# RiccZamboni/mepol

Measured on AMD Instinct MI355X. Metric: MEPOL epoch wall-clock (C3: N=200000, d=29, k=30; rollout excluded), lower is better.
Workload: dtype f64; 1 GPU; C3 Ant-shaped MEPOL epoch (k-NN + off-policy loop + final H); particles=200000, num_traj=400, traj_len=500, d=29, k=30, policy=29->[400, 300]->8 f64, parallelism=dp1

## Files before the change

### mepol_amd/csrc/policy_fwd.hip

```cpp
#include "mfma_f64.hpp"

namespace mepol {
namespace pfwd {

using mfma::d4;
using mfma::head_epilogue;
using mfma::kLog2Pi;
using mfma::kStdEps;

constexpr int BM = 64, BN = 320;
constexpr int WC = 4;
constexpr int FR = 2, FC = 5;
constexpr int kThreads = 512;
constexpr int KT = 16, KP = 18;
constexpr int CB = BN * (KT / 2), PB = CB / kThreads;
constexpr int kAChunk = 8;
static_assert(CB % kThreads == 0, "W2 k-tile chunks must divide the block");
static_assert(kThreads == BM * kAChunk, "head_epilogue: one thread per (row, action slot)");

template <int FP>
constexpr size_t lds_bytes() {
  return (2ull * BM * KP + 2ull * BN * KP + (size_t)(BM + 2 * KT) * (FP + 2)) * sizeof(double);
}

template <int FP, bool VEC>
__global__ __launch_bounds__(kThreads) void policy_fwd_kernel(
    const double* __restrict__ x, int64_t N, int F, const double* __restrict__ W1,
    const double* __restrict__ b1, int H1, const double* __restrict__ W2,
    const double* __restrict__ b2, int H2, const double* __restrict__ Wm,
    const double* __restrict__ bm, const double* __restrict__ log_std,
    const double* __restrict__ act, int A, double* __restrict__ h1_out,
    double* __restrict__ z2_out, double* __restrict__ mu_out, double* __restrict__ logp_out,
    uint16_t* __restrict__ mask_out) {
  constexpr int XP = FP + 2;
  extern __shared__ double lds[];
  double* sA = lds;
  double* sB = sA + 2 * BM * KP;
  double* sX = sB + 2 * BN * KP;
  double* sW = sX + BM * XP;
  const int tid = threadIdx.x, lane = tid & 63, wave = tid >> 6;
  const int wr = wave / WC, wc = wave % WC;
  const int fr = lane & 15, g = lane >> 4;
  const int64_t row0 = (int64_t)blockIdx.x * BM;
  const int nkt = (H1 + KT - 1) / KT;

  for (int e = tid; e < BM * FP; e += kThreads) {
    const int r = e / FP, f = e % FP;
    const int64_t rr = min<int64_t>(row0 + r, N - 1);
    const double v = x[rr * F + min(f, F - 1)];
    sX[r * XP + f] = (f < F && row0 + r < N) ? v : 0.0;
  }

  constexpr int PW = (KT * FP + kThreads - 1) / kThreads;
  double rw[PW];
  auto w1_load = [&](int kt) __attribute__((always_inline)) {
#pragma unroll
    for (int p = 0; p < PW; ++p) {
      const int e = tid + p * kThreads, r = e / FP, f = e % FP;
      rw[p] = W1[(int64_t)min(kt * KT + r, H1 - 1) * F + min(f, F - 1)];
    }
  };
  auto w1_store = [&](int kt) __attribute__((always_inline)) {
#pragma unroll
    for (int p = 0; p < PW; ++p) {
      const int e = tid + p * kThreads, r = e / FP, f = e % FP;
      if (e < KT * FP) sW[((kt & 1) * KT + r) * XP + f] = (kt * KT + r < H1 && f < F) ? rw[p] : 0.0;
    }
  };
  auto h1_gen = [&](int kt, int buf) __attribute__((always_inline)) {
    constexpr int NS = FP / 4, NCH = NS < 4 ? NS : 4;
    d4 hc[NCH];
#pragma unroll
    for (int u = 0; u < NCH; ++u) hc[u] = d4{0.0, 0.0, 0.0, 0.0};
    const double* xr = sX + (wave * 16 + fr) * XP + g;
    const double* wr1 = sW + ((kt & 1) * KT + fr) * XP + g;
#pragma unroll
    for (int s = 0; s < NS; ++s)
      hc[s % NCH] = __builtin_amdgcn_mfma_f64_16x16x4f64(xr[4 * s], wr1[4 * s], hc[s % NCH], 0,
                                                         0, 0);
    d4 h = hc[0];
#pragma unroll
    for (int u = 1; u < NCH; ++u) h += hc[u];
    const int c = kt * KT + fr;
    const double bc = c < H1 ? b1[c] : 0.0;
    const int mw = (H1 + 15) / 16;
#pragma unroll
    for (int q = 0; q < 4; ++q) {
      const int r = wave * 16 + g + 4 * q;
      const double v = c < H1 ? fmax(h[q] + bc, 0.0) : 0.0;
      sA[(buf * BM + r) * KP + fr] = v;
      if (c < H1 && row0 + r < N) h1_out[(row0 + r) * H1 + c] = v;
      const uint64_t bits = __ballot(v > 0.0);
      if (mask_out && fr == 0 && row0 + r < N)
        mask_out[(row0 + r) * mw + kt] = (uint16_t)(bits >> (16 * g));
    }
  };

  double2 rb[PB];
  auto b_load = [&](int kt) __attribute__((always_inline)) {
#pragma unroll
    for (int p = 0; p < PB; ++p) {
      const int ch = tid + p * kThreads, r = ch >> 3, k = kt * KT + 2 * (ch & 7);
      const double* row = W2 + (int64_t)min(r, H2 - 1) * H1;
      double2 v;
      if constexpr (VEC)
        v = *reinterpret_cast<const double2*>(row + min(k, H1 - 2));
      else
        v = double2{row[min(k, H1 - 1)], row[min(k + 1, H1 - 1)]};
      rb[p] = v;
    }
  };
  auto b_store = [&](int kt, int buf) __attribute__((always_inline)) {
#pragma unroll
    for (int p = 0; p < PB; ++p) {
      const int ch = tid + p * kThreads, r = ch >> 3, k = kt * KT + 2 * (ch & 7);
      double2 v = rb[p];
      if (r >= H2 || k >= H1) v = double2{0.0, 0.0};
      if (k + 1 >= H1) v.y = 0.0;
      *reinterpret_cast<double2*>(sB + (buf * BN + r) * KP + 2 * (ch & 7)) = v;
    }
  };

  d4 acc[FR][FC];
#pragma unroll
  for (int i = 0; i < FR; ++i)
#pragma unroll
    for (int j = 0; j < FC; ++j) acc[i][j] = d4{0.0, 0.0, 0.0, 0.0};

  b_load(0);
  w1_load(0);
  w1_store(0);
  if (nkt > 1) {
    w1_load(1);
    w1_store(1);
  }
  __syncthreads();
  if (wave < 4) h1_gen(0, 0);
  b_store(0, 0);
  __syncthreads();
  for (int kt = 0; kt < nkt; ++kt) {
    const int buf = kt & 1;
    if (kt + 1 < nkt) {
      b_load(kt + 1);
      if (kt + 2 < nkt) w1_load(kt + 2);
      if (wave < 4) h1_gen(kt + 1, buf ^ 1);
    }
    double2 a[FR][2], b[FC][2];
#pragma unroll
    for (int i = 0; i < FR; ++i) {
      const double* p = sA + (buf * BM + wr * FR * 16 + i * 16 + fr) * KP + 4 * g;
      a[i][0] = *reinterpret_cast<const double2*>(p);
      a[i][1] = *reinterpret_cast<const double2*>(p + 2);
    }
#pragma unroll
    for (int j = 0; j < FC; ++j) {
      const double* p = sB + (buf * BN + wc * FC * 16 + j * 16 + fr) * KP + 4 * g;
      b[j][0] = *reinterpret_cast<const double2*>(p);
      b[j][1] = *reinterpret_cast<const double2*>(p + 2);
    }
#pragma unroll
    for (int s = 0; s < 4; ++s) {
#pragma unroll
      for (int i = 0; i < FR; ++i) {
        const double av = (s & 1) ? a[i][s >> 1].y : a[i][s >> 1].x;
#pragma unroll
        for (int j = 0; j < FC; ++j) {
          const double bv = (s & 1) ? b[j][s >> 1].y : b[j][s >> 1].x;
          acc[i][j] = __builtin_amdgcn_mfma_f64_16x16x4f64(av, bv, acc[i][j], 0, 0, 0);
        }
      }
    }
    if (kt + 1 < nkt) {
      b_store(kt + 1, buf ^ 1);
      if (kt + 2 < nkt) w1_store(kt + 2);
    }
    __syncthreads();
  }

  head_epilogue<FR, FC, kAChunk, WC, BM>(acc, row0, wr * FR * 16, wc, N, b2, H2, Wm, bm, log_std,
                                         act, A, z2_out, mu_out, logp_out, sB);
}

template <int FP, int RG>
__global__ __launch_bounds__(256) void layer1_kernel(const double* __restrict__ x, int64_t N,
                                                     int F, const double* __restrict__ W1,
                                                     const double* __restrict__ b1, int H1,
                                                     double* __restrict__ h1_out,
                                                     uint16_t* __restrict__ mask_out) {
  constexpr int NS = FP / 4;
  const int l = threadIdx.x & 63, fr = l & 15, g = l >> 4;
  const int64_t r0 = ((int64_t)blockIdx.x * 4 + (threadIdx.x >> 6)) * 16 * RG;
  if (r0 >= N) return;
  double xv[RG][NS];
#pragma unroll
  for (int rg = 0; rg < RG; ++rg) {
    const int64_t xr = min<int64_t>(r0 + 16 * rg + fr, N - 1);
#pragma unroll
    for (int s = 0; s < NS; ++s) {
      const int f = 4 * s + g;
      const double v = x[xr * F + min(f, F - 1)];
      xv[rg][s] = f < F ? v : 0.0;
    }
  }
  const int nkt = (H1 + 15) / 16, mw = nkt;
  double wv[2][NS], bc[2];
  auto loadw = [&](int b, int kt) __attribute__((always_inline)) {
    const int c = min(kt * 16 + fr, H1 - 1);
    const double* wr = W1 + (int64_t)c * F;
#pragma unroll
    for (int s = 0; s < NS; ++s) {
      const int f = 4 * s + g;
      const double v = wr[min(f, F - 1)];
      wv[b][s] = f < F ? v : 0.0;
    }
    bc[b] = b1[c];
  };
  auto tile = [&](int b, int kt) __attribute__((always_inline)) {
    if (kt + 1 < nkt) loadw(b ^ 1, kt + 1);
    d4 h[RG];
#pragma unroll
    for (int rg = 0; rg < RG; ++rg) h[rg] = d4{0.0, 0.0, 0.0, 0.0};
#pragma unroll
    for (int s = 0; s < NS; ++s)
#pragma unroll
      for (int rg = 0; rg < RG; ++rg)
        h[rg] = __builtin_amdgcn_mfma_f64_16x16x4f64(xv[rg][s], wv[b][s], h[rg], 0, 0, 0);
    const int c = kt * 16 + fr;
#pragma unroll
    for (int rg = 0; rg < RG; ++rg)
#pragma unroll
      for (int q = 0; q < 4; ++q) {
        const int64_t r = r0 + 16 * rg + g + 4 * q;
        const double v = c < H1 ? fmax(h[rg][q] + bc[b], 0.0) : 0.0;
        if (c < H1 && r < N) __builtin_nontemporal_store(v, h1_out + r * H1 + c);
        const uint64_t bits = __ballot(v > 0.0);
        if (mask_out && fr == 0 && r < N) mask_out[r * mw + kt] = (uint16_t)(bits >> (16 * g));
      }
  };
  loadw(0, 0);
  int kt = 0;
#pragma nounroll
  for (; kt + 1 < nkt; kt += 2) {
    tile(0, kt);
    tile(1, kt + 1);
  }
  if (kt < nkt) tile(0, kt);
}

namespace zh {
constexpr int FI = 5, NW = 4, NS = 2;
constexpr int kCUs = 256;
constexpr int kOcc = 2;
inline int pick_tile(int64_t n) {
  for (int tile = 16; tile < 64; tile *= 2)
    if ((n + tile - 1) / tile <= kCUs) return tile;
  return 64;
}
}

template <int FO>
__global__ __launch_bounds__(64 * zh::NW) __attribute__((amdgpu_waves_per_eu(zh::kOcc))) void z2_head_kernel(
    const double* __restrict__ h1, int64_t N, int H1, const double* __restrict__ W2,
    const double* __restrict__ b2, int H2, const double* __restrict__ Wm,
    const double* __restrict__ bm, const double* __restrict__ log_std,
    const double* __restrict__ act, int A, double* __restrict__ z2_out,
    double* __restrict__ mu_out, double* __restrict__ logp_out) {
  constexpr int FI = zh::FI, NW = zh::NW, NS = zh::NS, NL = FO + FI;
  constexpr int ZM = 16 * FO;
  __shared__ double sMu[NW * ZM * 4];
  const int tid = threadIdx.x, l = tid & 63, fr = l & 15, g = l >> 4;
  const int w = __builtin_amdgcn_readfirstlane(tid >> 6);
  const int64_t row0 = (int64_t)blockIdx.x * ZM;
  const int col0 = 16 * FI * w;
  const double* ap[FO];
  const double* bp[FI];
#pragma unroll
  for (int t = 0; t < FO; ++t) ap[t] = h1 + min<int64_t>(row0 + 16 * t + fr, N - 1) * H1 + 2 * g;
#pragma unroll
  for (int u = 0; u < FI; ++u) bp[u] = W2 + (int64_t)min(col0 + 16 * u + fr, H2 - 1) * H1 + 2 * g;
  d4 acc[FO][FI];
#pragma unroll
  for (int t = 0; t < FO; ++t)
#pragma unroll
    for (int u = 0; u < FI; ++u) acc[t][u] = d4{0.0, 0.0, 0.0, 0.0};
  const int nst = (H1 + 7) / 8, nfull = H1 / 8;
  double2 R[NS][NL];
  auto load = [&](double2 (&D)[NL], int st) __attribute__((always_inline)) {
    const int k = min(8 * st, H1 - 2 - 2 * g);
#pragma unroll
    for (int t = 0; t < FO; ++t) D[t] = *reinterpret_cast<const double2*>(ap[t] + k);
#pragma unroll
    for (int u = 0; u < FI; ++u) D[FO + u] = *reinterpret_cast<const double2*>(bp[u] + k);
  };
  auto mma = [&](const double2 (&D)[NL]) __attribute__((always_inline)) {
#pragma unroll
    for (int t = 0; t < FO; ++t)
#pragma unroll
      for (int u = 0; u < FI; ++u)
        acc[t][u] = __builtin_amdgcn_mfma_f64_16x16x4f64(D[t].x, D[FO + u].x, acc[t][u], 0, 0, 0);
#pragma unroll
    for (int t = 0; t < FO; ++t)
#pragma unroll
      for (int u = 0; u < FI; ++u)
        acc[t][u] = __builtin_amdgcn_mfma_f64_16x16x4f64(D[t].y, D[FO + u].y, acc[t][u], 0, 0, 0);
  };
  mfma::ring_k_loop<NS, false>(
      nfull, nst, [&](int p, int st) __attribute__((always_inline)) { load(R[p], st); },
      [&](int p, int st) __attribute__((always_inline)) {
        if (8 * st + 2 * g >= H1) {
#pragma unroll
          for (int v = 0; v < NL; ++v) R[p][v] = double2{0.0, 0.0};
        }
      },
      [&](int p) __attribute__((always_inline)) { mma(R[p]); });

  double b2v[FI];
#pragma unroll
  for (int u = 0; u < FI; ++u) {
    const int c = col0 + 16 * u + fr;
    b2v[u] = c < H2 ? b2[c] : -HUGE_VAL;
#pragma unroll
    for (int t = 0; t < FO; ++t)
#pragma unroll
      for (int q = 0; q < 4; ++q) {
        const int64_t r = row0 + 16 * t + g + 4 * q;
        if (c < H2 && r < N) z2_out[r * H2 + c] = acc[t][u][q];
      }
  }
  constexpr int AC = 4;
  const int er = tid >> 2, ea = tid & 3;
  double lp = 0.0;
  for (int a0 = 0; a0 < A; a0 += AC) {
    double wmv[FI][AC];
#pragma unroll
    for (int u = 0; u < FI; ++u) {
      const int c = col0 + 16 * u + fr;
#pragma unroll
      for (int a = 0; a < AC; ++a)
        wmv[u][a] = (c < H2 && a0 + a < A) ? Wm[(int64_t)(a0 + a) * H2 + c] : 0.0;
    }
#pragma unroll
    for (int t = 0; t < FO; ++t)
#pragma unroll
      for (int q = 0; q < 4; ++q) {
        double p[AC];
#pragma unroll
        for (int a = 0; a < AC; ++a) p[a] = 0.0;
#pragma unroll
        for (int u = 0; u < FI; ++u) {
          const double rv = fmax(acc[t][u][q] + b2v[u], 0.0);
#pragma unroll
          for (int a = 0; a < AC; ++a) p[a] = fma(rv, wmv[u][a], p[a]);
        }
        int comp;
        const double v = mfma::reduce_scatter_g<AC, 16>(p, fr, comp);
        if ((fr & 3) == 0) sMu[(w * ZM + 16 * t + g + 4 * q) * AC + comp] = v;
      }
    __syncthreads();
    {
      const int a = a0 + ea;
      const int64_t r = row0 + er;
      double term = 0.0;
      if (er < ZM && a < A && r < N) {
        double m = sMu[(0 * ZM + er) * AC + ea];
#pragma unroll
        for (int v = 1; v < NW; ++v) m += sMu[(v * ZM + er) * AC + ea];
        m += bm[a];
        const double lsa = log_std[a];
        const double sd = exp(lsa) + kStdEps;
        const double d = act[r * A + a] - m;
        mu_out[r * A + a] = m;
        term = -0.5 * (kLog2Pi + 2.0 * lsa + d * d / (sd * sd));
      }
      term += __shfl_xor(term, 2, kWave);
      term += __shfl_xor(term, 1, kWave);
      lp += term;
    }
    __syncthreads();
  }
  if (ea == 0 && er < ZM && row0 + er < N) logp_out[row0 + er] = lp;
}

#ifndef MEPOL_L1_RG
#define MEPOL_L1_RG 2
#endif
constexpr int kLayer1RowGroups = MEPOL_L1_RG;

template <int FP>
int launch_split(const double* x, int64_t n, int F, const double* W1, const double* b1, int H1,
                 const double* W2, const double* b2, int H2, const double* Wm, const double* bm,
                 const double* log_std, const double* act, int A, double* h1, double* z2,
                 double* mu, double* logp, uint16_t* mask, int row_tile, hipStream_t st) {
  const int tile = row_tile ? row_tile : zh::pick_tile(n);
  const unsigned blocks = (unsigned)((n + tile - 1) / tile);
  constexpr int RG = kLayer1RowGroups;
  hipLaunchKernelGGL((layer1_kernel<FP, RG>), dim3((unsigned)((n + 64 * RG - 1) / (64 * RG))),
                     dim3(256), 0, st, x, n, F, W1, b1, H1, h1, mask);
  MEPOL_CHECK_LAUNCH();
#define MEPOL_Z2(FOV)                                                                       \
  hipLaunchKernelGGL(z2_head_kernel<FOV>, dim3(blocks), dim3(64 * zh::NW), 0, st, h1, n, H1, W2, \
                     b2, H2, Wm, bm, log_std, act, A, z2, mu, logp)
  if (tile == 64)
    MEPOL_Z2(4);
  else if (tile == 32)
    MEPOL_Z2(2);
  else
    MEPOL_Z2(1);
#undef MEPOL_Z2
  MEPOL_CHECK_LAUNCH();
  return 0;
}

template <int FP, bool VEC>
int launch(const double* x, int64_t n, int F, const double* W1, const double* b1, int H1,
           const double* W2, const double* b2, int H2, const double* Wm, const double* bm,
           const double* log_std, const double* act, int A, double* h1, double* z2, double* mu,
           double* logp, uint16_t* mask, hipStream_t st) {
  MEPOL_HIP((max_dynamic_lds<policy_fwd_kernel<FP, VEC>>((int)lds_bytes<FP>())));
  const unsigned blocks = (unsigned)((n + BM - 1) / BM);
  hipLaunchKernelGGL((policy_fwd_kernel<FP, VEC>), dim3(blocks), dim3(kThreads), lds_bytes<FP>(), st,
                     x, n, F, W1, b1, H1, W2, b2, H2, Wm, bm, log_std, act, A, h1, z2, mu, logp,
                     mask);
  MEPOL_CHECK_LAUNCH();
  return 0;
}

}
}

static int policy_forward(const char* who, const double* x, int64_t n, int in_features,
                          const double* W1, const double* b1, int hidden0, const double* W2,
                          const double* b2, int hidden1, const double* Wm, const double* bm,
                          const double* log_std, const double* actions, int action_dim,
                          double* h1_out, double* z2_out, double* mu_out, double* logp_out,
                          uint16_t* h1_mask_out, int row_tile, void* stream) {
  using namespace mepol::pfwd;
  if (n < 0 || in_features <= 0 || in_features > 64 || hidden0 <= 0 || hidden1 <= 0 ||
      hidden1 > BN || action_dim <= 0 || !x || !W1 || !b1 || !W2 || !b2 || !Wm || !bm ||
      !log_std || !actions || !h1_out || !z2_out || !mu_out || !logp_out ||
      ((uintptr_t)W2 & 15)) {
    mepol::set_error("%s: bad arguments (in_features <= 64, hidden1 <= %d)", who, BN);
    return mepol::kErrBadArg;
  }
  if (row_tile != 0 && row_tile != 64 && row_tile != 32 && row_tile != 16) {
    mepol::set_error("%s: row_tile %d (0 = automatic, 64, 32 or 16)", who, row_tile);
    return mepol::kErrBadArg;
  }
  const bool split = hidden0 % 2 == 0 && ((uintptr_t)h1_out & 15) == 0;
  if (!split && row_tile != 0 && row_tile != 64) {
    mepol::set_error("%s: the one-kernel form (odd hidden0) has 64-row blocks only, not %d", who,
                     row_tile);
    return mepol::kErrUnsupported;
  }
  if (n == 0) return 0;
  hipStream_t st = (hipStream_t)stream;
#define MEPOL_PF(FPV)                                                                        \
  {                                                                                          \
  if (split)                                                                                 \
    return launch_split<FPV>(x, n, in_features, W1, b1, hidden0, W2, b2, hidden1, Wm, bm,     \
                             log_std, actions, action_dim, h1_out, z2_out, mu_out, logp_out, \
                             h1_mask_out, row_tile, st);                                     \
  return (hidden0 % 2 == 0 && hidden0 >= 2)                                                  \
             ? launch<FPV, true>(x, n, in_features, W1, b1, hidden0, W2, b2, hidden1, Wm, bm, \
                                 log_std, actions, action_dim, h1_out, z2_out, mu_out,        \
                                 logp_out, h1_mask_out, st)                                   \
             : launch<FPV, false>(x, n, in_features, W1, b1, hidden0, W2, b2, hidden1, Wm,    \
                                  bm, log_std, actions, action_dim, h1_out, z2_out, mu_out,   \
                                  logp_out, h1_mask_out, st);                                  \
  }
  if (in_features <= 4) MEPOL_PF(4);
  if (in_features <= 8) MEPOL_PF(8);
  if (in_features <= 16) MEPOL_PF(16);
  if (in_features <= 32) MEPOL_PF(32);
  if (in_features <= 48) MEPOL_PF(48);
  MEPOL_PF(64);
#undef MEPOL_PF
}

extern "C" int mepol_policy_forward(const double* x, int64_t n, int in_features,
                                    const double* W1, const double* b1, int hidden0,
                                    const double* W2, const double* b2, int hidden1,
                                    const double* Wm, const double* bm, const double* log_std,
                                    const double* actions, int action_dim, double* h1_out,
                                    double* z2_out, double* mu_out, double* logp_out,
                                    void* stream) {
  return policy_forward("mepol_policy_forward", x, n, in_features, W1, b1, hidden0, W2, b2,
                        hidden1, Wm, bm, log_std, actions, action_dim, h1_out, z2_out, mu_out,
                        logp_out, nullptr, 0, stream);
}

extern "C" int mepol_policy_forward_masked(const double* x, int64_t n, int in_features,
                                           const double* W1, const double* b1, int hidden0,
                                           const double* W2, const double* b2, int hidden1,
                                           const double* Wm, const double* bm,
                                           const double* log_std, const double* actions,
                                           int action_dim, double* h1_out, double* z2_out,
                                           double* mu_out, double* logp_out,
                                           uint16_t* h1_mask_out, void* stream) {
  if (!h1_mask_out) {
    mepol::set_error("mepol_policy_forward_masked: h1_mask_out is null");
    return mepol::kErrBadArg;
  }
  return policy_forward("mepol_policy_forward_masked", x, n, in_features, W1, b1, hidden0, W2,
                        b2, hidden1, Wm, bm, log_std, actions, action_dim, h1_out, z2_out,
                        mu_out, logp_out, h1_mask_out, 0, stream);
}

extern "C" int mepol_policy_forward_tiled(const double* x, int64_t n, int in_features,
                                          const double* W1, const double* b1, int hidden0,
                                          const double* W2, const double* b2, int hidden1,
                                          const double* Wm, const double* bm,
                                          const double* log_std, const double* actions,
                                          int action_dim, double* h1_out, double* z2_out,
                                          double* mu_out, double* logp_out,
                                          uint16_t* h1_mask_out, int row_tile, void* stream) {
  return policy_forward("mepol_policy_forward_tiled", x, n, in_features, W1, b1, hidden0, W2, b2,
                        hidden1, Wm, bm, log_std, actions, action_dim, h1_out, z2_out, mu_out,
                        logp_out, h1_mask_out, row_tile, stream);
}

extern "C" int mepol_policy_forward_plan_info(int64_t n, int in_features, int hidden0,
                                              int hidden1, int* row_tile) {
  using namespace mepol::pfwd;
  if (n <= 0 || in_features <= 0 || in_features > 64 || hidden0 <= 0 || hidden1 <= 0 ||
      hidden1 > BN || !row_tile) {
    mepol::set_error("mepol_policy_forward_plan_info: bad arguments (in_features <= 64, "
                     "hidden1 <= %d)", BN);
    return mepol::kErrBadArg;
  }
  *row_tile = hidden0 % 2 == 0 ? zh::pick_tile(n) : BM;
  return 0;
}
```

Measured before the change: 0.09789 s/epoch.

## Add fast path to layer1 kernel with packed mask staging and 32-bit offsets

Adds a full-tile fast path to the layer-1 MFMA kernel that skips per-row bounds checks. It uses 32-bit byte offsets relative to the wave's row base and sets an occupancy hint through amdgpu_waves_per_eu. The relu mask words are staged in LDS per wave and then copied to global memory as 16-byte vectors, replacing scattered 2-byte stores. The aim is to cut address arithmetic, register pressure and uncoalesced mask writes, at the cost of more code complexity, dynamic shared memory, and 32-bit offset limits guarded by an H1 size check.

```diff
diff --git a/mepol_amd/csrc/policy_fwd.hip b/mepol_amd/csrc/policy_fwd.hip
--- a/mepol_amd/csrc/policy_fwd.hip
+++ b/mepol_amd/csrc/policy_fwd.hip
@@ -1,3 +1,5 @@
+#include <type_traits>
+
 #include "mfma_f64.hpp"
 
 namespace mepol {
@@ -181,15 +183,33 @@
                                          act, A, z2_out, mu_out, logp_out, sB);
 }
 
-template <int FP, int RG>
-__global__ __launch_bounds__(256) void layer1_kernel(const double* __restrict__ x, int64_t N,
-                                                     int F, const double* __restrict__ W1,
-                                                     const double* __restrict__ b1, int H1,
-                                                     double* __restrict__ h1_out,
-                                                     uint16_t* __restrict__ mask_out) {
+namespace l1s {
+constexpr int kFast = 1, kPack = 4, kDiet = 8;
+constexpr int kPackMaxWords = 128;
+constexpr int kMaxH1 = 1 << 20;
+constexpr int occ(int FP, int RG, int OPT) {
+  return !(OPT & kDiet) ? 1 : (RG + 2) * FP / 2 <= 64 ? 4 : 2;
+}
+template <int M>
+struct mode {
+  static constexpr int value = M;
+};
+}
+
+template <int FP, int RG, int OPT>
+__global__ __launch_bounds__(256) __attribute__((amdgpu_waves_per_eu(l1s::occ(FP, RG, OPT))))
+void layer1_kernel(const double* __restrict__ x, int64_t N, int F, const double* __restrict__ W1,
+                   const double* __restrict__ b1, int H1, double* __restrict__ h1_out,
+                   uint16_t* __restrict__ mask_out, int pack) {
   constexpr int NS = FP / 4;
+  constexpr bool kFast = (OPT & l1s::kFast) != 0,
+                 kPack = kFast && (OPT & l1s::kPack), kDiet = kFast && (OPT & l1s::kDiet);
+  static_assert(RG == 1 || RG == 2 || RG == 4, "a lane per row of the wave for the mask word");
+  extern __shared__ uint4 l1_slab[];
   const int l = threadIdx.x & 63, fr = l & 15, g = l >> 4;
-  const int64_t r0 = ((int64_t)blockIdx.x * 4 + (threadIdx.x >> 6)) * 16 * RG;
+  const int w = kDiet ? __builtin_amdgcn_readfirstlane((int)(threadIdx.x >> 6))
+                      : (int)(threadIdx.x >> 6);
+  const int64_t r0 = ((int64_t)blockIdx.x * 4 + w) * 16 * RG;
   if (r0 >= N) return;
   double xv[RG][NS];
 #pragma unroll
@@ -203,48 +223,144 @@
     }
   }
   const int nkt = (H1 + 15) / 16, mw = nkt;
+  using Off = typename std::conditional<kDiet, uint32_t, int64_t>::type;
+  const int64_t rb = kDiet ? 0 : r0;
+  const char* wb = reinterpret_cast<const char*>(W1);
+  char* hb = reinterpret_cast<char*>(kDiet ? h1_out + r0 * H1 : h1_out);
+  char* mb = reinterpret_cast<char*>(kDiet ? mask_out + r0 * mw : mask_out);
+  const Off wlast = (Off)8 * ((Off)H1 * (Off)F - 1);
   double wv[2][NS], bc[2];
   auto loadw = [&](int b, int kt) __attribute__((always_inline)) {
     const int c = min(kt * 16 + fr, H1 - 1);
-    const double* wr = W1 + (int64_t)c * F;
+    const Off co = (Off)8 * ((Off)c * (Off)F + (Off)g);
+#pragma unroll
+    for (int s = 0; s < NS; ++s)
+      wv[b][s] = *reinterpret_cast<const double*>(wb + min<Off>(co + (Off)(32 * s), wlast));
+    bc[b] = b1[c];
+  };
+  auto mul = [&](int b, d4 (&h)[RG]) __attribute__((always_inline)) {
+#pragma unroll
+    for (int rg = 0; rg < RG; ++rg) h[rg] = d4{0.0, 0.0, 0.0, 0.0};
 #pragma unroll
     for (int s = 0; s < NS; ++s) {
-      const int f = 4 * s + g;
-      const double v = wr[min(f, F - 1)];
-      wv[b][s] = f < F ? v : 0.0;
-    }
-    bc[b] = b1[c];
-  };
-  auto tile = [&](int b, int kt) __attribute__((always_inline)) {
-    if (kt + 1 < nkt) loadw(b ^ 1, kt + 1);
+      const double ws = 4 * s + g < F ? wv[b][s] : 0.0;
+#pragma unroll
+      for (int rg = 0; rg < RG; ++rg)
+        h[rg] = __builtin_amdgcn_mfma_f64_16x16x4f64(xv[rg][s], ws, h[rg], 0, 0, 0);
+    }
+  };
+  auto tile = [&](int b, int kt, uint16_t* slab) __attribute__((always_inline)) {
+    loadw(b ^ 1, min(kt + 1, nkt - 1));
+    __builtin_amdgcn_sched_barrier(0);
     d4 h[RG];
-#pragma unroll
-    for (int rg = 0; rg < RG; ++rg) h[rg] = d4{0.0, 0.0, 0.0, 0.0};
-#pragma unroll
-    for (int s = 0; s < NS; ++s)
+    mul(b, h);
+    __builtin_amdgcn_sched_barrier(0);
+    int lt = threadIdx.x;
+    if constexpr (kDiet) asm volatile("" : "+v"(lt));
+    const int fr = lt & 15, g = (lt >> 4) & 3;
+    const Off po = (Off)8 * (Off)((rb + g) * H1 + fr), pm = (Off)2 * (Off)((rb + g) * mw);
+    const int c = kt * 16 + fr;
+#pragma unroll
+    for (int rg = 0; rg < RG; ++rg)
+#pragma unroll
+      for (int q = 0; q < 4; ++q) {
+        const int rl = 16 * rg + 4 * q;
+        const bool rok = r0 + rl + g < N;
+        const double v = c < H1 ? fmax(h[rg][q] + bc[b], 0.0) : 0.0;
+        if (c < H1 && rok)
+          __builtin_nontemporal_store(
+              v, reinterpret_cast<double*>(hb + (po + (Off)8 * ((Off)rl * (Off)H1 + (Off)(16 * kt)))));
+        const uint64_t bits = __ballot(v > 0.0);
+        if (mask_out && fr == 0 && rok) {
+          const uint16_t word = (uint16_t)(bits >> (16 * g));
+          if (slab)
+            slab[(rl + g) * mw + kt] = word;
+          else
+            *reinterpret_cast<uint16_t*>(mb + (pm + (Off)2 * (Off)(rl * mw + kt))) = word;
+        }
+      }
+  };
+  loadw(0, 0);
+  if constexpr (kFast) {
+    if (r0 + 16 * RG <= N) {
+      const Off ho = (Off)8 * (Off)((rb + g) * H1 + fr);
+      char* hbs[RG][4];
 #pragma unroll
       for (int rg = 0; rg < RG; ++rg)
-        h[rg] = __builtin_amdgcn_mfma_f64_16x16x4f64(xv[rg][s], wv[b][s], h[rg], 0, 0, 0);
-    const int c = kt * 16 + fr;
-#pragma unroll
-    for (int rg = 0; rg < RG; ++rg)
-#pragma unroll
-      for (int q = 0; q < 4; ++q) {
-        const int64_t r = r0 + 16 * rg + g + 4 * q;
-        const double v = c < H1 ? fmax(h[rg][q] + bc[b], 0.0) : 0.0;
-        if (c < H1 && r < N) __builtin_nontemporal_store(v, h1_out + r * H1 + c);
-        const uint64_t bits = __ballot(v > 0.0);
-        if (mask_out && fr == 0 && r < N) mask_out[r * mw + kt] = (uint16_t)(bits >> (16 * g));
-      }
-  };
-  loadw(0, 0);
+#pragma unroll
+        for (int q = 0; q < 4; ++q) hbs[rg][q] = hb + 8 * (int64_t)(16 * rg + 4 * q) * H1;
+      const int j = fr & (4 * RG - 1), mrow = 16 * (j >> 2) + g + 4 * (j & 3);
+      const Off mo = (Off)2 * (Off)((rb + mrow) * mw);
+      uint16_t* slab = reinterpret_cast<uint16_t*>(l1_slab) + w * 16 * RG * mw;
+      const int nft = H1 / 16;
+      auto ftile = [&](int b, int kt, auto mk) __attribute__((always_inline)) {
+        constexpr int MK = decltype(mk)::value;
+        loadw(b ^ 1, min(kt + 1, nkt - 1));
+        __builtin_amdgcn_sched_barrier(0);
+        d4 h[RG];
+        mul(b, h);
+        __builtin_amdgcn_sched_barrier(0);
+        const Off hk = ho + (Off)(128 * kt);
+        uint64_t sel = 0;
+#pragma unroll
+        for (int rg = 0; rg < RG; ++rg) {
+#pragma unroll
+          for (int q = 0; q < 4; ++q) {
+            const double v = fmax(h[rg][q] + bc[b], 0.0);
+            if constexpr (MK != 0) {
+              const uint64_t bits = __ballot(v > 0.0);
+              sel = j == 4 * rg + q ? bits : sel;
+            }
+            __builtin_nontemporal_store(v, reinterpret_cast<double*>(hbs[rg][q] + hk));
+          }
+        }
+        if constexpr (MK != 0) {
+          const uint16_t word = (uint16_t)(sel >> (16 * g));
+          if constexpr (MK == 2)
+            slab[mrow * mw + kt] = word;
+          else
+            *reinterpret_cast<uint16_t*>(mb + (mo + (Off)(2 * kt))) = word;
+        }
+      };
+      auto run = [&](auto mk) __attribute__((always_inline)) {
+        constexpr int MK = decltype(mk)::value;
+        uint16_t* sl = MK == 2 ? slab : nullptr;
+        int kt = 0;
+#pragma nounroll
+        for (; kt + 2 <= nft; kt += 2) {
+          ftile(0, kt, mk);
+          ftile(1, kt + 1, mk);
+        }
+        if (kt < nft) {
+          ftile(0, kt, mk);
+          if (kt + 1 < nkt) tile(1, kt + 1, sl);
+        } else if (kt < nkt) {
+          tile(0, kt, sl);
+        }
+        if constexpr (MK == 2) {
+          __builtin_amdgcn_fence(__ATOMIC_ACQ_REL, "wavefront");
+          __builtin_amdgcn_wave_barrier();
+          const uint4* s4 = reinterpret_cast<const uint4*>(slab);
+          uint4* m4 = reinterpret_cast<uint4*>(mask_out + r0 * mw);
+          for (int i = l; i < 2 * RG * mw; i += 64) m4[i] = s4[i];
+        }
+      };
+      if (!mask_out)
+        run(l1s::mode<0>{});
+      else if (kPack && pack)
+        run(l1s::mode<2>{});
+      else
+        run(l1s::mode<1>{});
+      return;
+    }
+  }
   int kt = 0;
 #pragma nounroll
   for (; kt + 1 < nkt; kt += 2) {
-    tile(0, kt);
-    tile(1, kt + 1);
-  }
-  if (kt < nkt) tile(0, kt);
+    tile(0, kt, nullptr);
+    tile(1, kt + 1, nullptr);
+  }
+  if (kt < nkt) tile(0, kt, nullptr);
 }
 
 namespace zh {
@@ -385,6 +501,10 @@
 #define MEPOL_L1_RG 2
 #endif
 constexpr int kLayer1RowGroups = MEPOL_L1_RG;
+#ifndef MEPOL_L1_STORE
+#define MEPOL_L1_STORE 13
+#endif
+constexpr int kLayer1Store = MEPOL_L1_STORE;
 
 template <int FP>
 int launch_split(const double* x, int64_t n, int F, const double* W1, const double* b1, int H1,
@@ -393,9 +513,17 @@
                  double* mu, double* logp, uint16_t* mask, int row_tile, hipStream_t st) {
   const int tile = row_tile ? row_tile : zh::pick_tile(n);
   const unsigned blocks = (unsigned)((n + tile - 1) / tile);
-  constexpr int RG = kLayer1RowGroups;
-  hipLaunchKernelGGL((layer1_kernel<FP, RG>), dim3((unsigned)((n + 64 * RG - 1) / (64 * RG))),
-                     dim3(256), 0, st, x, n, F, W1, b1, H1, h1, mask);
+  constexpr int RG = kLayer1RowGroups, OPT = kLayer1Store;
+  const int mw = (H1 + 15) / 16;
+  const int pack = (OPT & l1s::kPack) && mask && ((uintptr_t)mask & 15) == 0 &&
+                   mw <= l1s::kPackMaxWords;
+  const dim3 grid((unsigned)((n + 64 * RG - 1) / (64 * RG)));
+  if (H1 <= l1s::kMaxH1)
+    hipLaunchKernelGGL((layer1_kernel<FP, RG, OPT>), grid, dim3(256),
+                       pack ? (size_t)128 * RG * mw : 0, st, x, n, F, W1, b1, H1, h1, mask, pack);
+  else
+    hipLaunchKernelGGL((layer1_kernel<FP, RG, 0>), grid, dim3(256), 0, st, x, n, F, W1, b1, H1,
+                       h1, mask, 0);
   MEPOL_CHECK_LAUNCH();
 #define MEPOL_Z2(FOV)                                                                       \
   hipLaunchKernelGGL(z2_head_kernel<FOV>, dim3(blocks), dim3(64 * zh::NW), 0, st, h1, n, H1, W2, \
```

Result: no change. 0.09696 s/epoch, median of 6 (-1.0%).
